# CrawlScript/tf_geometric

Measured on NVIDIA H100. Metric: edges/sec GCN+GAT fwd on 2.4M-node/123M-edge synthetic; %HBM roofline, higher is better.
Workload: dtype f32

## Files before the change

### tf_geometric_b200/csrc/gemm_proj.cu

```cuda
#include "common.cuh"
#include <type_traits>

namespace tfgk {
namespace proj {

constexpr int BM = 128;
constexpr int BK = 32;
constexpr int kUN = 128;
constexpr int kThreads = 256;
constexpr int kApitch = BK + 4;
constexpr int kStageBytes = BM * kApitch * 4;
constexpr int kMaxBlocks = 4;
constexpr int kMaxParts = 8;

struct Params {
    const float *A[kMaxParts];
    int64_t lda, part_rows;
    int first_tile;
    int M, K, kpad, nb, tiles_m, n_groups;
    const float *B[kMaxBlocks]; int64_t ldb[kMaxBlocks];
    const float *bias[kMaxBlocks]; int act[kMaxBlocks]; int ncols[kMaxBlocks]; int transb[kMaxBlocks];
    float *C[kMaxBlocks]; int64_t ldc[kMaxBlocks];
};

struct Plan {
    uint32_t kpad, b_bytes, ring_off, stages, total;
    explicit Plan(int K) {
        kpad = (uint32_t)((K + 7) / 8) * 8;
        b_bytes = (uint32_t)kUN * kpad * 4u;
        ring_off = 2u * b_bytes + kUN * 4u;
        const uint32_t budget = 227u * 1024u;
        stages = 0;
        for (uint32_t st = 4; st >= 2; --st)
            if (ring_off + st * kStageBytes <= budget) { stages = st; break; }
        total = ring_off + stages * kStageBytes;
    }
};

__device__ __forceinline__ uint32_t smem_u32(const void *p) { return (uint32_t)__cvta_generic_to_shared(p); }

__device__ __forceinline__ uint32_t w_offset(int n, int k, int kpad) {
    return (uint32_t)(n >> 3) * (uint32_t)(kpad * 32) + (uint32_t)(k >> 2) * 128u + (uint32_t)(n & 7) * 16u + (uint32_t)(k & 3) * 4u;
}

__device__ __forceinline__ uint64_t make_desc(uint32_t saddr, uint32_t sbo_bytes) {
    uint64_t d = 0;
    d |= (uint64_t)((saddr & 0x3FFFFu) >> 4);
    d |= (uint64_t)(128u >> 4) << 16;
    d |= (uint64_t)(sbo_bytes >> 4) << 32;
    return d;
}

__device__ __forceinline__ void split_tf32(float a, uint32_t &hi, uint32_t &lo) {
    const float lim = __uint_as_float(0x7F7FEFFFu);
    hi = (__float_as_uint(fminf(fmaxf(a, -lim), lim)) + 0x1000u) & 0xFFFFE000u;
    lo = __float_as_uint(a - __uint_as_float(hi));
}

__device__ __forceinline__ void cp_async16_zfill(uint32_t dst, const void *src, uint32_t src_bytes) {
    asm volatile("cp.async.cg.shared.global [%0], [%1], 16, %2;" ::"r"(dst), "l"(src), "r"(src_bytes) : "memory");
}

__device__ __forceinline__ void wgmma_fence() { asm volatile("wgmma.fence.sync.aligned;" ::: "memory"); }
__device__ __forceinline__ void wgmma_commit() { asm volatile("wgmma.commit_group.sync.aligned;" ::: "memory"); }
__device__ __forceinline__ void wgmma_wait_all() { asm volatile("wgmma.wait_group.sync.aligned 0;" ::: "memory"); }

__device__ __forceinline__ void wgmma_m64n128k8(float (&d)[64], const uint32_t (&a)[4], uint64_t b_desc, uint32_t accumulate) {
    asm volatile(
        "{\n\t.reg .pred p;\n\t"
        "setp.ne.b32 p, %69, 0;\n\t"
        "wgmma.mma_async.sync.aligned.m64n128k8.f32.tf32.tf32 "
        "{%0, %1, %2, %3, %4, %5, %6, %7, %8, %9, %10, %11, %12, %13, %14, %15, "
        "%16, %17, %18, %19, %20, %21, %22, %23, %24, %25, %26, %27, %28, %29, %30, %31, "
        "%32, %33, %34, %35, %36, %37, %38, %39, %40, %41, %42, %43, %44, %45, %46, %47, "
        "%48, %49, %50, %51, %52, %53, %54, %55, %56, %57, %58, %59, %60, %61, %62, %63}, "
        "{%64, %65, %66, %67}, %68, p, 1, 1;\n\t}"
        : "+f"(d[0]), "+f"(d[1]), "+f"(d[2]), "+f"(d[3]), "+f"(d[4]), "+f"(d[5]), "+f"(d[6]), "+f"(d[7]),
          "+f"(d[8]), "+f"(d[9]), "+f"(d[10]), "+f"(d[11]), "+f"(d[12]), "+f"(d[13]), "+f"(d[14]), "+f"(d[15]),
          "+f"(d[16]), "+f"(d[17]), "+f"(d[18]), "+f"(d[19]), "+f"(d[20]), "+f"(d[21]), "+f"(d[22]), "+f"(d[23]),
          "+f"(d[24]), "+f"(d[25]), "+f"(d[26]), "+f"(d[27]), "+f"(d[28]), "+f"(d[29]), "+f"(d[30]), "+f"(d[31]),
          "+f"(d[32]), "+f"(d[33]), "+f"(d[34]), "+f"(d[35]), "+f"(d[36]), "+f"(d[37]), "+f"(d[38]), "+f"(d[39]),
          "+f"(d[40]), "+f"(d[41]), "+f"(d[42]), "+f"(d[43]), "+f"(d[44]), "+f"(d[45]), "+f"(d[46]), "+f"(d[47]),
          "+f"(d[48]), "+f"(d[49]), "+f"(d[50]), "+f"(d[51]), "+f"(d[52]), "+f"(d[53]), "+f"(d[54]), "+f"(d[55]),
          "+f"(d[56]), "+f"(d[57]), "+f"(d[58]), "+f"(d[59]), "+f"(d[60]), "+f"(d[61]), "+f"(d[62]), "+f"(d[63])
        : "r"(a[0]), "r"(a[1]), "r"(a[2]), "r"(a[3]), "l"(b_desc), "r"(accumulate)
        : "memory");
}

__device__ __forceinline__ int tile_index(const Params &p, int group, int it) {
    int tl = group + it * p.n_groups + p.first_tile;
    return tl >= p.tiles_m ? tl - p.tiles_m : tl;
}

template <int STAGES>
__global__ void __launch_bounds__(kThreads, 1) gemm_proj_kernel(const Params p) {
    extern __shared__ __align__(128) uint8_t smem[];
    const int tid = threadIdx.x, lane = tid & 31, warp = tid >> 5;
    const int cb = blockIdx.x % p.nb, group = blockIdx.x / p.nb;
    const int kpad = p.kpad;
    const uint32_t b_bytes = (uint32_t)kUN * kpad * 4u;
    uint8_t *w_hi = smem, *w_lo = smem + b_bytes;
    float *s_bias = reinterpret_cast<float *>(smem + 2 * b_bytes);
    uint8_t *ring = smem + 2 * b_bytes + kUN * 4;
    const uint32_t ring_addr = smem_u32(ring);

    const int ncols = p.ncols[cb];
    const int my_tiles = group < p.tiles_m ? (p.tiles_m - group + p.n_groups - 1) / p.n_groups : 0;
    const int kb_per_tile = (p.K + BK - 1) / BK;
    const int total = my_tiles * kb_per_tile;

    auto load_stage = [&](int j) {
        if (j < total) {
            const int64_t row0 = (int64_t)tile_index(p, group, j / kb_per_tile) * BM;
            const int part = (int)(row0 / p.part_rows);
            const float *a_tile = p.A[part] + (row0 - (int64_t)part * p.part_rows) * p.lda;
            const int rows = (int)min((int64_t)BM, (int64_t)p.M - row0);
            const int k0 = (j % kb_per_tile) * BK;
            const uint32_t dst0 = ring_addr + (uint32_t)(j % STAGES) * kStageBytes;
            const int ch = tid & 7, gk = k0 + ch * 4;
            const uint32_t bytes = gk < p.K ? (uint32_t)min(16, (p.K - gk) * 4) : 0u;
#pragma unroll
            for (int i = 0; i < (BM * BK / 4) / kThreads; ++i) {
                const int r = (tid >> 3) + i * (kThreads / 8);
                const bool ok = r < rows && bytes != 0;
                cp_async16_zfill(dst0 + (uint32_t)(r * kApitch + ch * 4) * 4u, ok ? a_tile + (int64_t)r * p.lda + gk : p.A[0],
                                 ok ? bytes : 0u);
            }
        }
        asm volatile("cp.async.commit_group;" ::: "memory");
    };

#pragma unroll
    for (int s = 0; s < STAGES - 1; ++s) load_stage(s);

    {
        const float *B = p.B[cb];
        const int64_t ldb = p.ldb[cb];
        const bool tb = p.transb[cb] != 0;
        for (int idx = tid; idx < kUN * kpad; idx += kThreads) {
            int n, k;
            if (tb) { n = idx / kpad; k = idx % kpad; } else { k = idx / kUN; n = idx % kUN; }
            const float w = (n < ncols && k < p.K) ? (tb ? B[(int64_t)n * ldb + k] : B[(int64_t)k * ldb + n]) : 0.0f;
            uint32_t hi, lo;
            split_tf32(w, hi, lo);
            const uint32_t off = w_offset(n, k, kpad);
            *reinterpret_cast<uint32_t *>(w_hi + off) = hi;
            *reinterpret_cast<uint32_t *>(w_lo + off) = lo;
        }
        if (tid < kUN) s_bias[tid] = (p.bias[cb] != nullptr && tid < ncols) ? p.bias[cb][tid] : 0.0f;
    }
    asm volatile("fence.proxy.async.shared::cta;" ::: "memory");
    __syncthreads();

    const uint32_t w_hi_addr = smem_u32(w_hi), w_lo_addr = smem_u32(w_lo), sbo = (uint32_t)kpad * 32u;
    const int frag_row = (warp >> 2) * 64 + (warp & 3) * 16 + (lane >> 2);
    const int frag_col = lane & 3;
    const int act = p.act[cb];
    float *C = p.C[cb];
    const int64_t ldc = p.ldc[cb];
    const bool vec2 = (ldc % 2) == 0 && (reinterpret_cast<uintptr_t>(C) & 7u) == 0;
    float acc[64];
#pragma unroll
    for (int i = 0; i < 64; ++i) acc[i] = 0.0f;

    uint32_t ah[2][BK / 8][4], al[2][BK / 8][4];
    auto stage = [&](auto parity, int j) {
        constexpr int P = decltype(parity)::value;
        asm volatile("cp.async.wait_group %0;" ::"n"(STAGES - 2) : "memory");
        __syncthreads();
        load_stage(j + STAGES - 1);
        const int kb = j % kb_per_tile;
        const float *As = reinterpret_cast<const float *>(ring + (size_t)(j % STAGES) * kStageBytes);
#pragma unroll
        for (int ks = 0; ks < BK / 8; ++ks) {
            const float *a_r0 = As + frag_row * kApitch + ks * 8 + frag_col;
            const float *a_r8 = a_r0 + 8 * kApitch;
            split_tf32(a_r0[0], ah[P][ks][0], al[P][ks][0]);
            split_tf32(a_r8[0], ah[P][ks][1], al[P][ks][1]);
            split_tf32(a_r0[4], ah[P][ks][2], al[P][ks][2]);
            split_tf32(a_r8[4], ah[P][ks][3], al[P][ks][3]);
        }
        wgmma_wait_all();
        wgmma_fence();
#pragma unroll
        for (int ks = 0; ks < BK / 8; ++ks) {
            const int kg = kb * BK + ks * 8;
            if (kg < kpad) {
                const uint32_t koff = (uint32_t)(kg >> 2) * 128u;
                const uint64_t dh = make_desc(w_hi_addr + koff, sbo), dl = make_desc(w_lo_addr + koff, sbo);
                wgmma_m64n128k8(acc, al[P][ks], dh, (kb | ks) != 0);
                wgmma_m64n128k8(acc, ah[P][ks], dl, 1u);
                wgmma_m64n128k8(acc, ah[P][ks], dh, 1u);
            }
        }
        wgmma_commit();
        if (kb == kb_per_tile - 1) {
            wgmma_wait_all();
            const int64_t row0 = (int64_t)tile_index(p, group, j / kb_per_tile) * BM + frag_row;
#pragma unroll
            for (int h = 0; h < 2; ++h) {
                const int64_t row = row0 + 8 * h;
                if (row < p.M) {
                    float *crow = C + row * ldc;
#pragma unroll
                    for (int nb8 = 0; nb8 < kUN / 8; ++nb8) {
                        const int col = nb8 * 8 + 2 * frag_col;
                        const float v0 = apply_act(acc[4 * nb8 + 2 * h] + s_bias[col], act);
                        const float v1 = apply_act(acc[4 * nb8 + 2 * h + 1] + s_bias[col + 1], act);
                        if (vec2 && col + 1 < ncols) {
                            *reinterpret_cast<float2 *>(crow + col) = make_float2(v0, v1);
                        } else {
                            if (col < ncols) crow[col] = v0;
                            if (col + 1 < ncols) crow[col + 1] = v1;
                        }
                    }
                }
            }
        }
    };
    for (int j = 0; j < total; j += 2) {
        stage(std::integral_constant<int, 0>(), j);
        if (j + 1 < total) stage(std::integral_constant<int, 1>(), j + 1);
    }
    wgmma_wait_all();
    asm volatile("cp.async.wait_group 0;" ::: "memory");
}

template <int STAGES>
static int launch(const Params &p, int grid, uint32_t smem_bytes, cudaStream_t st) {
    TFGK_CUDA(ensure_dynamic_smem(gemm_proj_kernel<STAGES>, smem_bytes));
    gemm_proj_kernel<STAGES><<<grid, kThreads, smem_bytes, st>>>(p);
    TFGK_LAUNCH_CHECK();
    return TFGK_OK;
}

}
}

using namespace tfgk;

extern "C" int tfgk_gemm_proj_f32(const float *const *A_parts, int32_t n_parts, int64_t part_rows, int64_t lda,
                                  int32_t M, int32_t K, const tfgk_proj_block *blocks, int32_t n_blocks,
                                  int32_t first_part, int32_t max_ctas, void *stream) {
    TFGK_CHECK_ARG(A_parts != nullptr && blocks != nullptr, "gemm_proj: null argument");
    TFGK_CHECK_ARG(n_parts >= 1 && n_parts <= proj::kMaxParts, "gemm_proj: n_parts=%d not in [1, %d]", n_parts, proj::kMaxParts);
    TFGK_CHECK_ARG(n_blocks >= 1 && n_blocks <= proj::kMaxBlocks, "gemm_proj: n_blocks=%d not in [1, %d]", n_blocks, proj::kMaxBlocks);
    TFGK_CHECK_ARG(M >= 0 && K >= 1, "gemm_proj: bad size (M=%d, K=%d)", M, K);
    TFGK_CHECK_ARG(first_part >= 0 && first_part < n_parts, "gemm_proj: first_part=%d out of range", first_part);
    if (M == 0) return TFGK_OK;
    if (n_parts > 1)
        TFGK_CHECK_ARG(part_rows > 0 && part_rows % proj::BM == 0 && (int64_t)n_parts * part_rows >= M,
                       "gemm_proj: part_rows=%lld must be a positive multiple of %d covering M=%d", (long long)part_rows, proj::BM, M);
    if (K > 512 || (lda % 4) != 0 || lda < K) return TFGK_ERR_UNSUPPORTED;
    proj::Params p;
    for (int i = 0; i < proj::kMaxParts; ++i) {
        p.A[i] = A_parts[i < n_parts ? i : 0];
        if (!aligned16(p.A[i]) || p.A[i] == nullptr) return i < n_parts && A_parts[i] == nullptr
            ? set_error(TFGK_ERR_INVALID_ARGUMENT, "gemm_proj: A part %d is null", i) : TFGK_ERR_UNSUPPORTED;
    }
    p.lda = lda; p.part_rows = n_parts > 1 ? part_rows : (int64_t)1 << 40;
    p.M = M; p.K = K; p.nb = n_blocks;
    p.tiles_m = (int)ceil_div64(M, proj::BM);
    p.first_tile = n_parts > 1 ? (int)((int64_t)first_part * part_rows / proj::BM) : 0;
    if (p.first_tile >= p.tiles_m) p.first_tile = 0;
    for (int b = 0; b < proj::kMaxBlocks; ++b) {
        const tfgk_proj_block &blk = blocks[b < n_blocks ? b : 0];
        if (b < n_blocks) {
            TFGK_CHECK_ARG(blk.B != nullptr && blk.C != nullptr, "gemm_proj: block %d has a null operand", b);
            TFGK_CHECK_ARG(blk.ncols >= 1 && blk.ldb >= (blk.transB ? K : blk.ncols) && blk.ldc >= blk.ncols,
                           "gemm_proj: block %d has bad sizes", b);
            TFGK_CHECK_ARG(blk.act == TFGK_ACT_NONE || blk.act == TFGK_ACT_RELU, "gemm_proj: unknown activation %d", blk.act);
            if (blk.ncols > proj::kUN) return TFGK_ERR_UNSUPPORTED;
        }
        p.B[b] = blk.B; p.ldb[b] = blk.ldb; p.bias[b] = blk.bias; p.act[b] = blk.act; p.ncols[b] = blk.ncols;
        p.transb[b] = blk.transB;
        p.C[b] = blk.C; p.ldc[b] = blk.ldc;
    }
    const proj::Plan L(K);
    if (L.stages == 0) return TFGK_ERR_UNSUPPORTED;
    p.kpad = (int)L.kpad;
    int dev = 0, sms = 0;
    TFGK_CUDA(cudaGetDevice(&dev));
    TFGK_CUDA(cudaDeviceGetAttribute(&sms, cudaDevAttrMultiProcessorCount, dev));
    if (max_ctas > 0 && max_ctas < sms) sms = max_ctas;
    int n_groups = sms / n_blocks;
    if (n_groups < 1) n_groups = 1;
    if (n_groups > p.tiles_m) n_groups = p.tiles_m;
    p.n_groups = n_groups;
    const int grid = n_groups * n_blocks;
    cudaStream_t st = as_stream(stream);
    if (L.stages >= 4) return proj::launch<4>(p, grid, L.total, st);
    if (L.stages == 3) return proj::launch<3>(p, grid, L.total, st);
    return proj::launch<2>(p, grid, L.total, st);
}
```

Before: 3.580 billion.

## Warp-specialize projection GEMM with producer warp and mbarrier-pipelined deep ring

After: 3.575 billion (median of 6 runs). Within noise of the previous version (-0.1%).

```diff
diff --git a/tf_geometric_b200/csrc/gemm_proj.cu b/tf_geometric_b200/csrc/gemm_proj.cu
--- a/tf_geometric_b200/csrc/gemm_proj.cu
+++ b/tf_geometric_b200/csrc/gemm_proj.cu
@@ -5,19 +5,26 @@
 namespace proj {
 
 constexpr int BM = 128;
+constexpr int WM = 64;
 constexpr int BK = 32;
 constexpr int kUN = 128;
-constexpr int kThreads = 256;
+constexpr int kConsumers = 256;
+constexpr int kThreads = kConsumers + 32;
 constexpr int kApitch = BK + 4;
-constexpr int kStageBytes = BM * kApitch * 4;
+constexpr int kStageBytes = WM * kApitch * 4;
+constexpr int kMinStages = 4;
+constexpr int kMaxStages = 16;
+constexpr int kBarBytes = 2 * kMaxStages * 8;
 constexpr int kMaxBlocks = 4;
 constexpr int kMaxParts = 8;
+
+constexpr int kBarW = 1, kBarTurn = 2;
 
 struct Params {
     const float *A[kMaxParts];
     int64_t lda, part_rows;
     int first_tile;
-    int M, K, kpad, nb, tiles_m, n_groups;
+    int M, K, kpad, nb, tiles_m, n_groups, stages;
     const float *B[kMaxBlocks]; int64_t ldb[kMaxBlocks];
     const float *bias[kMaxBlocks]; int act[kMaxBlocks]; int ncols[kMaxBlocks]; int transb[kMaxBlocks];
     float *C[kMaxBlocks]; int64_t ldc[kMaxBlocks];
@@ -28,11 +35,11 @@
     explicit Plan(int K) {
         kpad = (uint32_t)((K + 7) / 8) * 8;
         b_bytes = (uint32_t)kUN * kpad * 4u;
-        ring_off = 2u * b_bytes + kUN * 4u;
+        ring_off = 2u * b_bytes + kUN * 4u + kBarBytes;
         const uint32_t budget = 227u * 1024u;
-        stages = 0;
-        for (uint32_t st = 4; st >= 2; --st)
-            if (ring_off + st * kStageBytes <= budget) { stages = st; break; }
+        stages = ring_off < budget ? (budget - ring_off) / kStageBytes : 0u;
+        if (stages > (uint32_t)kMaxStages) stages = kMaxStages;
+        if (stages < (uint32_t)kMinStages) stages = 0;
         total = ring_off + stages * kStageBytes;
     }
 };
@@ -61,9 +68,33 @@
     asm volatile("cp.async.cg.shared.global [%0], [%1], 16, %2;" ::"r"(dst), "l"(src), "r"(src_bytes) : "memory");
 }
 
+__device__ __forceinline__ void mbar_init(uint32_t bar, uint32_t count) {
+    asm volatile("mbarrier.init.shared::cta.b64 [%0], %1;" ::"r"(bar), "r"(count) : "memory");
+}
+__device__ __forceinline__ void mbar_arrive(uint32_t bar) {
+    asm volatile("mbarrier.arrive.shared::cta.b64 _, [%0];" ::"r"(bar) : "memory");
+}
+__device__ __forceinline__ void mbar_arrive_on_cp_async(uint32_t bar) {
+    asm volatile("cp.async.mbarrier.arrive.noinc.shared::cta.b64 [%0];" ::"r"(bar) : "memory");
+}
+__device__ __forceinline__ void mbar_wait(uint32_t bar, uint32_t parity) {
+    asm volatile(
+        "{\n\t.reg .pred done;\n\t"
+        "WAIT:\n\t"
+        "mbarrier.try_wait.parity.shared::cta.b64 done, [%0], %1;\n\t"
+        "@!done bra WAIT;\n\t}" ::"r"(bar), "r"(parity) : "memory");
+}
+__device__ __forceinline__ void named_sync(int id, int threads) {
+    asm volatile("bar.sync %0, %1;" ::"r"(id), "r"(threads) : "memory");
+}
+__device__ __forceinline__ void named_arrive(int id, int threads) {
+    asm volatile("bar.arrive %0, %1;" ::"r"(id), "r"(threads) : "memory");
+}
+
 __device__ __forceinline__ void wgmma_fence() { asm volatile("wgmma.fence.sync.aligned;" ::: "memory"); }
 __device__ __forceinline__ void wgmma_commit() { asm volatile("wgmma.commit_group.sync.aligned;" ::: "memory"); }
-__device__ __forceinline__ void wgmma_wait_all() { asm volatile("wgmma.wait_group.sync.aligned 0;" ::: "memory"); }
+template <int N>
+__device__ __forceinline__ void wgmma_wait() { asm volatile("wgmma.wait_group.sync.aligned %0;" ::"n"(N) : "memory"); }
 
 __device__ __forceinline__ void wgmma_m64n128k8(float (&d)[64], const uint32_t (&a)[4], uint64_t b_desc, uint32_t accumulate) {
     asm volatile(
@@ -92,52 +123,65 @@
     return tl >= p.tiles_m ? tl - p.tiles_m : tl;
 }
 
-template <int STAGES>
 __global__ void __launch_bounds__(kThreads, 1) gemm_proj_kernel(const Params p) {
     extern __shared__ __align__(128) uint8_t smem[];
-    const int tid = threadIdx.x, lane = tid & 31, warp = tid >> 5;
+    const int tid = threadIdx.x, lane = tid & 31;
     const int cb = blockIdx.x % p.nb, group = blockIdx.x / p.nb;
-    const int kpad = p.kpad;
+    const int kpad = p.kpad, S = p.stages;
     const uint32_t b_bytes = (uint32_t)kUN * kpad * 4u;
     uint8_t *w_hi = smem, *w_lo = smem + b_bytes;
     float *s_bias = reinterpret_cast<float *>(smem + 2 * b_bytes);
-    uint8_t *ring = smem + 2 * b_bytes + kUN * 4;
-    const uint32_t ring_addr = smem_u32(ring);
-
-    const int ncols = p.ncols[cb];
+    const uint32_t bars = smem_u32(smem + 2 * b_bytes + kUN * 4);
+    uint8_t *ring = smem + 2 * b_bytes + kUN * 4 + kBarBytes;
+    auto full = [&](int s) { return bars + 8u * (uint32_t)s; };
+    auto empty = [&](int s) { return bars + 8u * (uint32_t)(kMaxStages + s); };
+
     const int my_tiles = group < p.tiles_m ? (p.tiles_m - group + p.n_groups - 1) / p.n_groups : 0;
     const int kb_per_tile = (p.K + BK - 1) / BK;
-    const int total = my_tiles * kb_per_tile;
-
-    auto load_stage = [&](int j) {
-        if (j < total) {
-            const int64_t row0 = (int64_t)tile_index(p, group, j / kb_per_tile) * BM;
-            const int part = (int)(row0 / p.part_rows);
-            const float *a_tile = p.A[part] + (row0 - (int64_t)part * p.part_rows) * p.lda;
-            const int rows = (int)min((int64_t)BM, (int64_t)p.M - row0);
-            const int k0 = (j % kb_per_tile) * BK;
-            const uint32_t dst0 = ring_addr + (uint32_t)(j % STAGES) * kStageBytes;
-            const int ch = tid & 7, gk = k0 + ch * 4;
+    const int total = 2 * my_tiles * kb_per_tile;
+
+    if (tid == 0) {
+        for (int s = 0; s < S; ++s) {
+            mbar_init(full(s), 32);
+            mbar_init(empty(s), 4);
+        }
+    }
+    __syncthreads();
+
+    if (tid >= kConsumers) {
+        const int ch = lane & 7;
+        const uint32_t ring_addr = smem_u32(ring);
+        for (int j = 0; j < total; ++j) {
+            const int s = j % S, h = j / kb_per_tile, kb = j - h * kb_per_tile;
+            mbar_wait(empty(s), ((uint32_t)(j / S) & 1u) ^ 1u);
+            const int64_t tile0 = (int64_t)tile_index(p, group, h >> 1) * BM;
+            const int part = (int)(tile0 / p.part_rows);
+            const int64_t row0 = tile0 + (h & 1) * WM;
+            const float *a_half = p.A[part] + (row0 - (int64_t)part * p.part_rows) * p.lda;
+            const int64_t rows = (int64_t)p.M - row0;
+            const int gk = kb * BK + ch * 4;
             const uint32_t bytes = gk < p.K ? (uint32_t)min(16, (p.K - gk) * 4) : 0u;
-#pragma unroll
-            for (int i = 0; i < (BM * BK / 4) / kThreads; ++i) {
-                const int r = (tid >> 3) + i * (kThreads / 8);
+            const uint32_t dst0 = ring_addr + (uint32_t)s * kStageBytes;
+#pragma unroll
+            for (int i = 0; i < WM / 4; ++i) {
+                if (gk >= p.kpad) break;
+                const int r = (lane >> 3) + 4 * i;
                 const bool ok = r < rows && bytes != 0;
-                cp_async16_zfill(dst0 + (uint32_t)(r * kApitch + ch * 4) * 4u, ok ? a_tile + (int64_t)r * p.lda + gk : p.A[0],
+                cp_async16_zfill(dst0 + (uint32_t)(r * kApitch + ch * 4) * 4u, ok ? a_half + (int64_t)r * p.lda + gk : p.A[0],
                                  ok ? bytes : 0u);
             }
-        }
-        asm volatile("cp.async.commit_group;" ::: "memory");
-    };
-
-#pragma unroll
-    for (int s = 0; s < STAGES - 1; ++s) load_stage(s);
+            mbar_arrive_on_cp_async(full(s));
+        }
+        asm volatile("cp.async.wait_all;" ::: "memory");
+        return;
+    }
 
     {
         const float *B = p.B[cb];
         const int64_t ldb = p.ldb[cb];
         const bool tb = p.transb[cb] != 0;
-        for (int idx = tid; idx < kUN * kpad; idx += kThreads) {
+        const int ncols = p.ncols[cb];
+        for (int idx = tid; idx < kUN * kpad; idx += kConsumers) {
             int n, k;
             if (tb) { n = idx / kpad; k = idx % kpad; } else { k = idx / kUN; n = idx % kUN; }
             const float w = (n < ncols && k < p.K) ? (tb ? B[(int64_t)n * ldb + k] : B[(int64_t)k * ldb + n]) : 0.0f;
@@ -150,11 +194,13 @@
         if (tid < kUN) s_bias[tid] = (p.bias[cb] != nullptr && tid < ncols) ? p.bias[cb][tid] : 0.0f;
     }
     asm volatile("fence.proxy.async.shared::cta;" ::: "memory");
-    __syncthreads();
-
+    named_sync(kBarW, kConsumers);
+
+    const int wg = tid >> 7, warp = (tid >> 5) & 3;
     const uint32_t w_hi_addr = smem_u32(w_hi), w_lo_addr = smem_u32(w_lo), sbo = (uint32_t)kpad * 32u;
-    const int frag_row = (warp >> 2) * 64 + (warp & 3) * 16 + (lane >> 2);
+    const int frag_row = warp * 16 + (lane >> 2);
     const int frag_col = lane & 3;
+    const int ncols = p.ncols[cb];
     const int act = p.act[cb];
     float *C = p.C[cb];
     const int64_t ldc = p.ldc[cb];
@@ -164,23 +210,27 @@
     for (int i = 0; i < 64; ++i) acc[i] = 0.0f;
 
     uint32_t ah[2][BK / 8][4], al[2][BK / 8][4];
-    auto stage = [&](auto parity, int j) {
+    auto kblock = [&](auto parity, int j, int kb) {
         constexpr int P = decltype(parity)::value;
-        asm volatile("cp.async.wait_group %0;" ::"n"(STAGES - 2) : "memory");
-        __syncthreads();
-        load_stage(j + STAGES - 1);
-        const int kb = j % kb_per_tile;
-        const float *As = reinterpret_cast<const float *>(ring + (size_t)(j % STAGES) * kStageBytes);
+        const int s = j % S;
+        mbar_wait(full(s), (uint32_t)(j / S) & 1u);
+        const float *As = reinterpret_cast<const float *>(ring + (size_t)s * kStageBytes);
+        float a[BK / 8][4];
 #pragma unroll
         for (int ks = 0; ks < BK / 8; ++ks) {
+            if (kb * BK + ks * 8 >= kpad) break;
             const float *a_r0 = As + frag_row * kApitch + ks * 8 + frag_col;
             const float *a_r8 = a_r0 + 8 * kApitch;
-            split_tf32(a_r0[0], ah[P][ks][0], al[P][ks][0]);
-            split_tf32(a_r8[0], ah[P][ks][1], al[P][ks][1]);
-            split_tf32(a_r0[4], ah[P][ks][2], al[P][ks][2]);
-            split_tf32(a_r8[4], ah[P][ks][3], al[P][ks][3]);
-        }
-        wgmma_wait_all();
+            a[ks][0] = a_r0[0]; a[ks][1] = a_r8[0]; a[ks][2] = a_r0[4]; a[ks][3] = a_r8[4];
+        }
+        __syncwarp();
+        if (lane == 0) mbar_arrive(empty(s));
+        wgmma_wait<1>();
+#pragma unroll
+        for (int ks = 0; ks < BK / 8; ++ks)
+            if (kb * BK + ks * 8 < kpad)
+#pragma unroll
+                for (int e = 0; e < 4; ++e) split_tf32(a[ks][e], ah[P][ks][e], al[P][ks][e]);
         wgmma_fence();
 #pragma unroll
         for (int ks = 0; ks < BK / 8; ++ks) {
@@ -194,44 +244,40 @@
             }
         }
         wgmma_commit();
-        if (kb == kb_per_tile - 1) {
-            wgmma_wait_all();
-            const int64_t row0 = (int64_t)tile_index(p, group, j / kb_per_tile) * BM + frag_row;
-#pragma unroll
-            for (int h = 0; h < 2; ++h) {
-                const int64_t row = row0 + 8 * h;
-                if (row < p.M) {
-                    float *crow = C + row * ldc;
-#pragma unroll
-                    for (int nb8 = 0; nb8 < kUN / 8; ++nb8) {
-                        const int col = nb8 * 8 + 2 * frag_col;
-                        const float v0 = apply_act(acc[4 * nb8 + 2 * h] + s_bias[col], act);
-                        const float v1 = apply_act(acc[4 * nb8 + 2 * h + 1] + s_bias[col + 1], act);
-                        if (vec2 && col + 1 < ncols) {
-                            *reinterpret_cast<float2 *>(crow + col) = make_float2(v0, v1);
-                        } else {
-                            if (col < ncols) crow[col] = v0;
-                            if (col + 1 < ncols) crow[col + 1] = v1;
-                        }
+    };
+
+    if (wg == 1 && my_tiles > 0) named_arrive(kBarTurn + 0, kConsumers);
+    for (int t = 0; t < my_tiles; ++t) {
+        const int j0 = (2 * t + wg) * kb_per_tile;
+        named_sync(kBarTurn + wg, kConsumers);
+        for (int kb = 0; kb < kb_per_tile; kb += 2) {
+            kblock(std::integral_constant<int, 0>(), j0 + kb, kb);
+            if (kb + 1 < kb_per_tile) kblock(std::integral_constant<int, 1>(), j0 + kb + 1, kb + 1);
+        }
+        if (wg == 0 || t + 1 < my_tiles) named_arrive(kBarTurn + (wg ^ 1), kConsumers);
+        wgmma_wait<0>();
+        const int64_t row0 = (int64_t)tile_index(p, group, t) * BM + wg * WM + frag_row;
+#pragma unroll
+        for (int h = 0; h < 2; ++h) {
+            const int64_t row = row0 + 8 * h;
+            if (row < p.M) {
+                float *crow = C + row * ldc;
+#pragma unroll
+                for (int nb8 = 0; nb8 < kUN / 8; ++nb8) {
+                    const int col = nb8 * 8 + 2 * frag_col;
+                    const float2 b = *reinterpret_cast<const float2 *>(s_bias + col);
+                    const float v0 = apply_act(acc[4 * nb8 + 2 * h] + b.x, act);
+                    const float v1 = apply_act(acc[4 * nb8 + 2 * h + 1] + b.y, act);
+                    if (vec2 && col + 1 < ncols) {
+                        *reinterpret_cast<float2 *>(crow + col) = make_float2(v0, v1);
+                    } else {
+                        if (col < ncols) crow[col] = v0;
+                        if (col + 1 < ncols) crow[col + 1] = v1;
                     }
                 }
             }
         }
-    };
-    for (int j = 0; j < total; j += 2) {
-        stage(std::integral_constant<int, 0>(), j);
-        if (j + 1 < total) stage(std::integral_constant<int, 1>(), j + 1);
-    }
-    wgmma_wait_all();
-    asm volatile("cp.async.wait_group 0;" ::: "memory");
-}
-
-template <int STAGES>
-static int launch(const Params &p, int grid, uint32_t smem_bytes, cudaStream_t st) {
-    TFGK_CUDA(ensure_dynamic_smem(gemm_proj_kernel<STAGES>, smem_bytes));
-    gemm_proj_kernel<STAGES><<<grid, kThreads, smem_bytes, st>>>(p);
-    TFGK_LAUNCH_CHECK();
-    return TFGK_OK;
+    }
 }
 
 }
@@ -279,6 +325,7 @@
     const proj::Plan L(K);
     if (L.stages == 0) return TFGK_ERR_UNSUPPORTED;
     p.kpad = (int)L.kpad;
+    p.stages = (int)L.stages;
     int dev = 0, sms = 0;
     TFGK_CUDA(cudaGetDevice(&dev));
     TFGK_CUDA(cudaDeviceGetAttribute(&sms, cudaDevAttrMultiProcessorCount, dev));
@@ -289,7 +336,8 @@
     p.n_groups = n_groups;
     const int grid = n_groups * n_blocks;
     cudaStream_t st = as_stream(stream);
-    if (L.stages >= 4) return proj::launch<4>(p, grid, L.total, st);
-    if (L.stages == 3) return proj::launch<3>(p, grid, L.total, st);
-    return proj::launch<2>(p, grid, L.total, st);
-}
+    TFGK_CUDA(ensure_dynamic_smem(proj::gemm_proj_kernel, L.total));
+    proj::gemm_proj_kernel<<<grid, proj::kThreads, L.total, st>>>(p);
+    TFGK_LAUNCH_CHECK();
+    return TFGK_OK;
+}
```
